# l-tamas/Fiasco

Hardware: AMD Instinct MI355X
Metric: grayscale frames/sec encoded (higher is better)
Workload: dtype f32

## Files before the change

fiasco_amd/csrc/hip/enc_layout.inc:

```

static bool long_basis(const fa_wfa *w)
{
    if (!w) return false;
    if (w->basis_states > FC_MAXBASIS) return true;
    for (unsigned s = 0; s < w->basis_states; s++)
        for (unsigned l = 0; l < 2; l++) {
            unsigned e = 0;
            while (e < 6 && FA_INTO(w, s, l, e) != FA_NO_EDGE) e++;
            if (e > FA_MAXEDGES) return true;
        }
    return false;
}
static size_t bx_bytes(const fa_wfa *w) { return 16 + (size_t) w->basis_states * 80 + 72; }

static bool needs_hm_variant(const fa_cparams *cp)
{
    return cp->rpf.mantissa_bits > 5 || cp->dc_rpf.mantissa_bits > 5 || cp->d_rpf.mantissa_bits > 5 || cp->d_dc_rpf.mantissa_bits > 5;
}

static bool needs_gm_variant(const fa_job *job)
{
    const fa_cparams *cp = &job->cp;
    const bool delta_used = cp->prediction || job->frame_type != FA_I_FRAME;
    return cp->pool_kind != FA_POOL_RLE || cp->coeff_kind != FA_COEFF_ADAPTIVE
           || (delta_used && (cp->d_pool_kind != FA_POOL_RLE || cp->d_coeff_kind != FA_COEFF_ADAPTIVE));
}

static bool needs_big_variant(const fa_cparams *cp, const fa_wfa *basis)
{
    if (needs_hm_variant(cp)) return true;
    if (cp->prediction) return true;
    if (long_basis(basis)) return true;
    if (basis)
        for (unsigned s = 0; s < basis->basis_states; s++)
            for (unsigned l = 0; l < 2; l++)
                for (unsigned e = 0; e < 6 && FA_INTO(basis, s, l, e) != FA_NO_EDGE; e++)
                    if (e >= 3) return true;
    unsigned dcs = 1u << (1 + cp->dc_rpf.mantissa_bits), sy = 1u << (1 + cp->rpf.mantissa_bits);
    return cp->lc_min_level <= cp->images_level || cp->lc_max_level > 10 || cp->max_elements > 3
           || cp->second_domain_block || cp->check_for_underflow || cp->check_for_overflow || cp->full_search
           || (cp->lc_max_level - cp->lc_min_level + 1) * sy + dcs > FC_MAXCOEFF
           || (cp->level - cp->lc_min_level + 3 + cp->lc_max_level - cp->lc_min_level)
              * ((32 + 2 * ((cp->lc_max_level - cp->lc_min_level + 1) * sy + dcs) + 15) / 16) > FC_SNAP16_WIDE;
}

static bool needs_wide_variant(const fa_cparams *cp)
{
    unsigned dcs = 1u << (1 + cp->dc_rpf.mantissa_bits), sy = 1u << (1 + cp->rpf.mantissa_bits);
    const unsigned n16 = (32 + 2 * ((cp->lc_max_level - cp->lc_min_level + 1) * sy + dcs) + 15) / 16;
    const unsigned depths = cp->level - cp->lc_min_level + 3;
    return depths - 1 > FC_MAXDEPTH_NARROW
           || (depths + cp->lc_max_level - cp->lc_min_level) * n16 > FC_SNAP16_NARROW
           || depths * 4 * ((2 * cp->limit_level + 3) / 4) > FC_SNAPTM_NARROW;
}


struct Layout {
    size_t gram, gcol, diag, ipis, d5, d4, img, imgT, imgT4, norms, num, den, est, ipdo, used, tree, into, weight,
           final_d, level_of_state, domain_type, x, y, ycol, pool_states, pos, hits, ycol0, snap, pix16, total;
    size_t ipis_alt, d5_alt, d4_alt, pix_save, sv_gram, sv_img, sv_auto;
    size_t mv, past, future, mc_fwd, mc_bwd, pix_chroma;
    size_t coop;
    size_t bx;
    size_t gq, lginv;
    int    max_save;
};

static Layout make_layout(int P, int PA, int NL, int NS, int NA, int NI, int il, int low, size_t npix,
                          int max_save, int inter, int plevels, int color, bool tri, bool hm, int gm_states = 0)
{
    Layout L;
    memset(&L, 0, sizeof L);
    size_t o = 0;
    L.max_save = max_save;
#define CARVE(field, bytes) do { L.field = o; o = align_up(o + (bytes), 256); } while (0)
    CARVE(gram, tri ? (size_t) NL * ((size_t) P * (P + 1) / 2 + P) * 4 : (size_t) NL * P * P * 4);
    CARVE(gcol, tri ? (size_t) NL * FC_TRI_HOT * P * 4 : 0);
    CARVE(diag, (size_t) NL * P * 4);
    CARVE(ipis, (size_t) NS * P * 4);
    CARVE(d5, (size_t) NA * P * 4);
    CARVE(d4, low ? (size_t) 2 * NA * P * 4 : 0);
    CARVE(img, (size_t) P * NI * 4);
    CARVE(imgT, ((size_t) 1 << il) * P * 4);
    CARVE(imgT4, low ? ((size_t) 1 << (il - 1)) * P * 4 : 0);
    CARVE(norms, (size_t) NS * 4);
    CARVE(num, (size_t) P * 4);
    CARVE(den, (size_t) P * 4);
    CARVE(est, (size_t) P * 4);
    CARVE(ipdo, (size_t) FC_MAXED * P * 4);
    CARVE(used, (size_t) P);
    CARVE(tree, (size_t) 2 * PA * 2);
    CARVE(into, (size_t) 12 * PA * 2);
    CARVE(weight, (size_t) 12 * PA * 4);
    CARVE(final_d, (size_t) PA * 4);
    CARVE(level_of_state, (size_t) PA);
    CARVE(domain_type, (size_t) PA);
    CARVE(x, (size_t) 2 * PA * 2);
    CARVE(y, (size_t) 2 * PA * 2);
    CARVE(ycol, (size_t) 2 * PA);
    CARVE(mv, inter ? (size_t) 10 * PA * 2 : 0);
    CARVE(pool_states, (size_t) (P + 8) * 2);
    CARVE(pos, (size_t) (PA + 8) * 2);
    CARVE(hits, (size_t) (PA + 8) * 4);
    CARVE(ycol0, (size_t) 2 * PA);
    const size_t n16max = FC_N16(hm ? FC_MAXCOEFF_HM : FC_MAXCOEFF_BIG_STD);
    CARVE(snap, max_save ? (size_t) (FC_MAXDEPTH_BIG * 5 * n16max + FC_MAXDEPTH_BIG * 2 * 28) * 16
                         : (size_t) 26 * 2 * n16max * 16);
    CARVE(ipis_alt, max_save ? (size_t) NS * P * 4 : 0);
    CARVE(d5_alt, max_save ? (size_t) NA * P * 4 : 0);
    CARVE(d4_alt, max_save && low ? (size_t) 2 * NA * P * 4 : 0);
    CARVE(pix_save, max_save ? (size_t) (4096 + 128) * 4 : 0);
    CARVE(sv_gram, (size_t) max_save * NL * P * 4);
    CARVE(sv_img, (size_t) max_save * (NI + 48 + NL) * 4);
    CARVE(sv_auto, (size_t) max_save * sizeof(FcSavedRow));
    CARVE(past, inter ? npix * 2 : 0);
    CARVE(future, inter == 2 ? npix * 2 : 0);
    CARVE(mc_fwd, inter ? (size_t) plevels * 1024 * 4 : 0);
    CARVE(mc_bwd, inter ? (size_t) plevels * 1024 * 4 : 0);
    CARVE(pix_chroma, inter && color ? npix / 3 * 2 * 2 : 0);
    CARVE(coop, FC_COOP_HDR + ((size_t) (NS + 1) << il) * 4);
    CARVE(bx, FC_BX_BYTES);
    CARVE(gq, gm_states ? (size_t) FC_GQ_SLOTS * P * 2 : 0);
    CARVE(lginv, gm_states ? ((size_t) gm_states + 2) * 8 : 0);
    CARVE(pix16, npix * 2);
#undef CARVE
    L.total = o;
    return L;
}

static int device_supported(const fa_job *job, char *why, size_t n)
{
    const fa_cparams *cp = &job->cp;
    const bool window_reachable = (int) cp->p_max_level >= (int) cp->lc_min_level;
    if (job->frame_type != FA_I_FRAME && window_reachable
        && (!job->past || (job->frame_type == FA_B_FRAME && !job->future) || cp->search_range != 16)) {
        snprintf(why, n, "Motion search without a reference frame (frame pattern).");
        return 0;
    }
    if ((cp->prediction || job->frame_type != FA_I_FRAME) && (int) cp->p_max_level - (int) cp->lc_min_level + 1 > 9) {
        snprintf(why, n, "prediction over more than 9 block levels is not supported by the device coder (levels %u .. %u, frame type %d)",
                 cp->lc_min_level, cp->p_max_level, job->frame_type);
        return 0;
    }
    if (cp->images_level != 5 || cp->lc_min_level < 4) {
        snprintf(why, n, "device coder needs images_level 5 and min block level >= 4");
        return 0;
    }
    if (cp->lc_max_level > 12) { snprintf(why, n, "max block level > 12 is not supported by the device coder"); return 0; }
    if (cp->max_elements > 5) { snprintf(why, n, "more than 5 vectors per block are not supported by the device coder"); return 0; }
    {
        unsigned dcs = 1u << (1 + cp->dc_rpf.mantissa_bits), sy = 1u << (1 + cp->rpf.mantissa_bits);
        if ((cp->lc_max_level - cp->lc_min_level + 1) * sy + dcs > FC_MAXCOEFF_HM) {
            snprintf(why, n, "coefficient model too large for the device coder "
                             "(block levels x mantissa symbols > %d)", FC_MAXCOEFF_HM);
            return 0;
        }
    }
    if (cp->rpf.mantissa_bits > 8 || cp->dc_rpf.mantissa_bits > 8 || cp->d_rpf.mantissa_bits > 8 || cp->d_dc_rpf.mantissa_bits > 8) {
        snprintf(why, n, "RPF mantissa > 8 bits is not supported by the device coder");
        return 0;
    }
    if (long_basis(job->wfa)) {
        const fa_wfa *w = job->wfa;
        if (bx_bytes(w) > FC_BX_BYTES) { snprintf(why, n, "initial basis too large for the device coder"); return 0; }
        for (unsigned r = 0; r < w->basis_states * 2; r++) {
            unsigned e = r * 6;
            while (e < w->basis_states * 12 && w->into[e] != FA_NO_EDGE) e++;
            if (e >= w->basis_states * 12) { snprintf(why, n, "edge lists of the initial basis run on into the coder's states"); return 0; }
        }
    }
    return 1;
}
```

fiasco_amd/csrc/hip/enc_stage.inc:

```


struct FrameSlot {
    int      job;
    char    *base = nullptr;
    size_t   bytes = 0;
    int      slab_dev = -1;
    int      P = 0, PA = 0;
    int      floorP = 0, floorPA = 0;
    Layout   L;
    DevFrame F;
    bool     staged = false, done = false, big = false, rejected = false;
    bool     hm = false;
    bool     gm = false;
    std::vector<double> lginv_host;
    bool     wide_only = false;
    bool     tri = false;
    bool     borrow = false;
    bool     spec = false;
    std::vector<uint8_t> ycol_host;
    std::vector<int32_t> bx_host;
    const int16_t *ext_pix = nullptr;
    const int16_t *ext_next = nullptr;
    const fa_image *src = nullptr;
};
// ... 10 lines not shown
    int  ncu = 256;
    std::vector<size_t>   batch;
    std::vector<DevFrame> hf;
    FcTrace *d_trace = nullptr;
    bool inflight = false, launch_failed = false, broken = false;
    int  good = 0;
    std::vector<std::pair<size_t, size_t>> to_unpack;
    char  *pinned = nullptr;
    size_t pinned_bytes = 0;
    char  *d_pack[2] = { nullptr, nullptr };
    size_t d_pack_bytes[2] = { 0, 0 }, pack_need = 0;
    int    parity = 0;
    bool   packed = false, copy_pending = false;
    std::vector<size_t> pack_off;
    hipStream_t cstream = nullptr;
    char  *up_host = nullptr;
    size_t up_host_bytes = 0;
    bool   up_host_shared = false;
    char  *up_dev[2] = { nullptr, nullptr };
    size_t up_dev_bytes[2] = { 0, 0 };
    int    up_parity = 0;
    bool   up_pending = false;
    hipStream_t ustream = nullptr;
    hipEvent_t  ev_up = nullptr;
    char  *ic_tab = nullptr, *d_ic = nullptr;
    size_t ic_cap = 0;
    hipEvent_t  ev_ic = nullptr;
    char  *peer_buf = nullptr;
    size_t peer_bytes = 0;
    char   ic_failed[200] = "";
    int       lender0 = -1;
    Layout    qL;
    int       qP = 0, qPA = 0;
    bool      qbig = false, qtri = false;
    size_t    lenders = 0, borrowers = 0, lender_cap = 0;
    char     *qpix = nullptr;
    size_t    qpix_bytes = 0, qpix_used = 0;
    unsigned long long *d_ring = nullptr;
    size_t    ring_n = 0;
    unsigned *d_queue = nullptr;
    unsigned *d_ptrmask = nullptr;
    bool      ptrmask_ready = false;
    bool      no_coop = false, no_coop_done = false;
    FcCoop    coop_hdr;
    int       specG = 0;
    int       specH[2] = { 0, 0 };
    bool      no_app = false;
    DevFrame *d_vframes = nullptr;
    size_t    vframes_n = 0;
    char     *d_spec = nullptr;
    size_t    d_spec_bytes = 0, spec_ctl_span = 0;
    std::vector<size_t> spec_frames;
    size_t    spec_first[2] = { 0, 0 }, spec_n[2] = { 0, 0 };
};

static Build build_of(const Staged *S, const FrameSlot &fs, bool few)
{
    const bool wide_only = fs.P > 12 * 256 || fs.wide_only;
    if (fs.spec && S->specG >= 2 && !fs.borrow && !fs.tri && !fs.big && fs.P <= 12 * 1024)
        return wide_only ? B_SPEC_WIDE : B_SPEC;
    if (fs.gm) return B_BIG_GM;
    if (fs.hm) return B_BIG_HM;
    if (fs.tri) return B_WIDE_TRI;
    return (Build) ((fs.big ? B_BIG : B_DEFAULT) + (few || wide_only ? 1 : 0));
}

static size_t frames_per_cu(const FrameSlot &fs)
{
    static std::atomic<int> cache[N_BUILDS];
    const Build b = fs.gm ? B_BIG_GM : fs.hm ? B_BIG_HM
                  : (Build) ((fs.big ? B_BIG : B_DEFAULT) + (fs.P > 12 * 256 || fs.wide_only ? 1 : 0));
    int occ = cache[b].load(std::memory_order_relaxed);
    if (!occ) {
        occ = k_build[b].occupancy();
        if (occ < 1) occ = 1;
        cache[b].store(occ, std::memory_order_relaxed);
    }
    return (size_t) occ;
}

static inline const fa_image *slot_image(const Staged *S, const FrameSlot &fs)
{
    return fs.src ? fs.src : S->jobs[fs.job].image;
}

static void fill_frame(FrameSlot &fs, const fa_job *job)
{
    const fa_cparams *cp = &job->cp;
    const fa_wfa *w = job->wfa;
    DevFrame &F = fs.F;
    const Layout &L = fs.L;
    char *base = fs.base;
    memset(&F, 0, sizeof F);
    F.price = cp->price;
    F.lc_min = (int) cp->lc_min_level; F.lc_max = (int) cp->lc_max_level;
    F.images_level = (int) cp->images_level; F.max_elements = (int) cp->max_elements;
    const bool bxl = long_basis(w);
    {
        unsigned live = cp->max_elements;
        for (unsigned st = 0; st < (bxl ? 0u : w->basis_states); st++)
            for (unsigned l = 0; l < 2; l++) {
                unsigned e = 0;
                while (e < 6 && FA_INTO(w, st, l, e) != FA_NO_EDGE) e++;
                if (e > live) live = e;
            }
        F.maxe_live = (int) live;
    }
    F.level = (int) cp->level; F.width = (int) job->image->width; F.height = (int) job->image->height;
    F.pool_max = (int) cp->pool_max_states; F.limit_states = (int) cp->limit_states;
    F.ML = (int) cp->limit_level;
    F.rpf_mant = (int) cp->rpf.mantissa_bits; F.dc_mant = (int) cp->dc_rpf.mantissa_bits;
    F.rpf_range = cp->rpf.range; F.dc_range = cp->dc_rpf.range;
    F.P = fs.P; F.PA = fs.PA;
    F.gram_ls = fs.tri ? (unsigned) ((size_t) fs.P * (fs.P + 1) / 2 + fs.P) : (unsigned) fs.P * (unsigned) fs.P;
    F.color = job->image->color ? 1 : 0;
    F.chroma_cl_cap = (int) knob_int("FIASCO_AMD_CLMAX", 0);
    F.chroma_sparse = !fa_knob("FIASCO_AMD_CHROMA_FULL") && (cp->pool_kind == FA_POOL_RLE || cp->pool_kind == FA_POOL_ADAPTIVE || cp->pool_kind == FA_POOL_BASIS);
    F.chroma_max = (int) cp->chroma_max_states;
    F.chroma_decrease = cp->chroma_decrease;
    F.plane = (unsigned long long) job->image->width * job->image->height;
    F.gl0 = (int) (cp->lc_min_level < cp->images_level ? cp->lc_min_level : cp->images_level);
    F.NL = (int) cp->lc_max_level - F.gl0 + 1;
    F.second_domain_block = cp->second_domain_block ? 1 : 0;
    F.check_underflow = cp->check_for_underflow ? 1 : 0;
    F.check_overflow = cp->check_for_overflow ? 1 : 0;
    F.full_search = cp->full_search ? 1 : 0;
    F.NS = (int) fa_size_of_tree(cp->products_level);
    F.NA = 1 << (cp->lc_max_level - cp->images_level);
    F.NI = (int) fa_size_of_tree(cp->images_level);
    F.dcs = 1 << (1 + F.dc_mant); F.sy = 1 << (1 + F.rpf_mant);
    F.coeff_size = (F.lc_max - F.lc_min + 1) * F.sy + F.dcs;
    F.coeff_nt = F.lc_max - F.lc_min + 2;
    F.basis_states = (int) w->basis_states;
    F.bx = bxl ? (const int *) (base + L.bx) : nullptr;
    F.gm_pool[0] = (int) cp->pool_kind; F.gm_pool[1] = (int) cp->d_pool_kind;
    F.gm_coeff[0] = (int) cp->coeff_kind; F.gm_coeff[1] = (int) cp->d_coeff_kind;
    F.gq = fs.gm ? (int16_t *) (base + L.gq) : nullptr;
    F.lginv = fs.gm ? (const double *) (base + L.lginv) : nullptr;
    for (unsigned s = 0; s < (bxl ? 0u : w->basis_states); s++) {
        F.b_final[s] = w->final_distribution[s];
        F.b_dtype[s] = w->domain_type[s];
        for (int l = 0; l < 2; l++) {
            F.b_tree[s][l] = FA_TREE(w, s, l);
            for (int e = 0; e < 6; e++) {
                F.b_into[s][l][e] = FA_INTO(w, s, l, e);
                F.b_weight[s][l][e] = FA_WEIGHT(w, s, l, e);
                if (FA_INTO(w, s, l, e) == FA_NO_EDGE) break;
            }
        }
    }
    F.pix16 = (const int16_t *) (base + L.pix16);
    F.gram = (float *) (base + L.gram); F.diag = (float *) (base + L.diag);
    F.ipis = (float *) (base + L.ipis); F.d5 = (float *) (base + L.d5);
    F.gcol = (float *) (base + L.gcol);
    F.d4 = (float *) (base + L.d4); F.imgT4 = (float *) (base + L.imgT4);
    F.img = (float *) (base + L.img); F.imgT = (float *) (base + L.imgT);
    F.norms = (float *) (base + L.norms);
    F.num = (float *) (base + L.num); F.den = (float *) (base + L.den);
    F.est = (float *) (base + L.est); F.ipdo = (float *) (base + L.ipdo);
    F.used = (uint8_t *) (base + L.used);
    F.tree = (int16_t *) (base + L.tree); F.into = (int16_t *) (base + L.into);
    F.weight = (float *) (base + L.weight); F.final_d = (float *) (base + L.final_d);
    F.level_of_state = (uint8_t *) (base + L.level_of_state);
    F.domain_type = (uint8_t *) (base + L.domain_type);
    F.x = (uint16_t *) (base + L.x); F.y = (uint16_t *) (base + L.y);
    F.ycol = (uint8_t *) (base + L.ycol);
    F.ycol0 = job->ycol_carry ? (const uint8_t *) (base + L.ycol0) : nullptr;
    F.pool_states = (int16_t *) (base + L.pool_states);
    F.pos = (int16_t *) (base + L.pos);
    F.hits = (int *) (base + L.hits);
    F.snap_hbm = fs.big ? (void *) (base + L.snap) : nullptr;
    F.l2_keys = g_l2.d_keys; F.l2_vals = g_l2.d_vals; F.l2_mask = g_l2.mask;
    const int inter = job->frame_type != FA_I_FRAME;
    F.pred_on = cp->prediction || inter ? 1 : 0;
    F.pred_root = job->image->color ? inter : (cp->prediction || inter ? 1 : 0);
    F.search_range = (int) cp->search_range;
    F.mv = (int16_t *) (base + L.mv);
    F.past = (const int16_t *) (base + L.past); F.future = (const int16_t *) (base + L.future);
    F.coop = (FcCoop *) (base + L.coop);
    F.mc_fwd = (float *) (base + L.mc_fwd); F.mc_bwd = inter ? (float *) (base + L.mc_bwd) : nullptr;
    F.pix_chroma = (int16_t *) (base + L.pix_chroma);
    F.frame_type = job->frame_type;
    F.p_min = (int) cp->p_min_level; F.p_max = (int) cp->p_max_level;
    F.d_rpf_mant = (int) cp->d_rpf.mantissa_bits; F.d_dc_mant = (int) cp->d_dc_rpf.mantissa_bits;
    F.d_rpf_range = cp->d_rpf.range; F.d_dc_range = cp->d_dc_rpf.range;
    F.d_dcs = 1 << (1 + F.d_dc_mant); F.d_sy = 1 << (1 + F.d_rpf_mant);
    F.d_coeff_size = (F.lc_max - F.lc_min + 1) * F.d_sy + F.d_dcs;
    F.ipis_alt = (float *) (base + L.ipis_alt); F.d5_alt = (float *) (base + L.d5_alt);
    F.d4_alt = (float *) (base + L.d4_alt); F.pix_save = (float *) (base + L.pix_save);
    F.sv_gram = (float *) (base + L.sv_gram); F.sv_img = (float *) (base + L.sv_img);
    F.sv_auto = (FcSavedRow *) (base + L.sv_auto);
    F.max_save = L.max_save;
    F.slab_base = base; F.slab_bytes = L.total;
}

static void slot_layout(Staged *S, FrameSlot &fs)
{
    const fa_job *job = &S->jobs[fs.job];
    const fa_cparams *cp = &job->cp;
    int il = (int) cp->images_level;
    int low = cp->lc_min_level < cp->images_level;
    int NL = (int) (cp->lc_max_level - (low ? cp->lc_min_level : cp->images_level) + 1);
    int NS = (int) fa_size_of_tree(cp->products_level);
    int NA = 1 << (cp->lc_max_level - cp->images_level);
    int NI = (int) fa_size_of_tree(cp->images_level);
    size_t npix = (size_t) job->image->width * job->image->height;
    const int bands = job->image->color ? 3 : 1;
    int max_save = 0;
    const int inter = job->frame_type;
    if (cp->prediction || inter) {
        int span = (int) cp->p_max_level - (int) cp->lc_min_level + 1;
        max_save = 1 << (span < 1 ? 1 : span > 9 ? 9 : span);
    }
    fs.L = make_layout(fs.P, fs.PA, NL, NS, NA, NI, il, low, npix * bands, max_save, inter,
                       (int) cp->p_max_level - (int) cp->p_min_level + 1, job->image->color ? 1 : 0, fs.tri, fs.hm || fs.gm,
                       fs.gm ? (int) cp->limit_states : 0);
}


static bool queue_eligible(const Staged *S, const FrameSlot &fs)
{
    const fa_job *job = &S->jobs[fs.job];
    return job->frame_type == FA_I_FRAME && !job->ycol_carry && !fs.spec && !long_basis(job->wfa) && !fs.hm && !fs.gm && !fa_knob("FIASCO_AMD_NO_QUEUE");
}

static bool queue_layout(const Staged *S, const FrameSlot &fs)
{
    if (S->lender0 < 0) return false;
    return fs.P == S->qP && fs.PA == S->qPA && fs.big == S->qbig && fs.tri == S->qtri
           && memcmp(&fs.L, &S->qL, sizeof(Layout)) == 0;
}

static int stage_borrower(Staged *S, FrameSlot &fs, size_t frames_left)
{
    fa_job *job = &S->jobs[fs.job];
    const FrameSlot &ref = S->slots[S->lender0];
    const size_t npix = (size_t) job->image->width * job->image->height;
    const int bands = job->image->color ? 3 : 1;
    const size_t need = align_up(npix * bands * 2, 256);
    if (!S->qpix && !fs.ext_pix) {
        size_t bytes = need * frames_left;
        if (hipMalloc((void **) &S->qpix, bytes) != hipSuccess) { S->qpix = nullptr; (void) hipGetLastError(); return 0; }
        S->qpix_bytes = bytes; S->qpix_used = 0;
    }
    if (!fs.ext_pix && S->qpix_used + need > S->qpix_bytes) return 0;
    fs.base = ref.base;
    fill_frame(fs, job);
    fs.base = nullptr; fs.bytes = 0;
    fs.borrow = true;
    if (fs.ext_pix) {
        fs.F.pix16 = fs.ext_pix;
        S->borrowers++;
        fs.staged = true;
        return 1;
    }
    fs.ext_pix = (const int16_t *) (S->qpix + S->qpix_used);
    fs.F.pix16 = fs.ext_pix;
    for (int b = 0; b < bands; b++)
        if (hipMemcpyAsync(S->qpix + S->qpix_used + (size_t) b * npix * 2, slot_image(S, fs)->pixels[b], npix * 2,
                           hipMemcpyHostToDevice, S->stream) != hipSuccess) {
            snprintf(job->errmsg, sizeof job->errmsg, "HIP error: pixel upload failed");
            fs.borrow = false; fs.ext_pix = nullptr;
            return 0;
        }
    S->qpix_used += need;
    S->borrowers++;
    fs.staged = true;
    return 1;
}

static bool upload_reference(Staged *S, const FrameSlot &fs, const fa_image *ref, size_t off, int here)
{
    const fa_job *job = &S->jobs[fs.job];
    const size_t npix = (size_t) job->image->width * job->image->height;
    const int bands = job->image->color ? 3 : 1;
    for (int b = 0; b < bands; b++)
        if ((ref->dev && ref->dev_id == here
             ? hipMemcpyAsync(fs.base + off + (size_t) b * npix * 2, (const int16_t *) ref->dev + (size_t) b * npix, npix * 2,
                              hipMemcpyDeviceToDevice, S->stream)
             : hipMemcpyAsync(fs.base + off + (size_t) b * npix * 2, ref->pixels[b], npix * 2,
                              hipMemcpyHostToDevice, S->stream)) != hipSuccess)
            return false;
    return true;
}

static int stage_slot(Staged *S, FrameSlot &fs)
{
    fa_job *job = &S->jobs[fs.job];
    const fa_cparams *cp = &job->cp;
    const size_t npix = (size_t) job->image->width * job->image->height;
    const int bands = job->image->color ? 3 : 1;
    slot_layout(S, fs);
    fs.base = slab_acquire(fs.L.total, &fs.bytes, &fs.slab_dev);
    if (fs.base && fa_knob("FIASCO_AMD_POISON"))
        (void) hipMemsetAsync(fs.base, (int) knob_int("FIASCO_AMD_POISON", 0), fs.L.total, S->stream);
    if (!fs.base) {
        snprintf(job->errmsg, sizeof job->errmsg, "out of HBM: frame needs %.2f GiB", fs.L.total / 1073741824.0);
        return 0;
    }
    auto give_up = [&](const char *msg) {
        snprintf(job->errmsg, sizeof job->errmsg, "%s", msg);
        slab_release(fs.base, fs.bytes, fs.slab_dev); fs.base = nullptr;
        return 0;
    };
    fill_frame(fs, job);
    const bool hmx = fs.hm || fs.gm;
// ... 324 lines not shown
```

fiasco_amd/csrc/hip/fc_config.inc:

```

#ifndef FC_VARIANT_WIDE
#define FC_VARIANT_WIDE 0
#endif
#if FC_VARIANT_WIDE
#ifndef FC_WIDE_B
#define FC_WIDE_B 512
#endif
#define B       FC_WIDE_B
#if defined(FC_VARIANT_BIG) && FC_VARIANT_BIG
#define FC_KREG 12
#elif !defined(FC_KREG)
#define FC_KREG (9216 / FC_WIDE_B)
#endif
#else
#define B       FC_BLOCK
#define FC_KREG 12
#endif
#ifndef FC_VARIANT_BIG
#define FC_VARIANT_BIG 0
#endif
#if FC_HM && !(FC_VARIANT_BIG && FC_VARIANT_WIDE)
#error "FC_HM is a variant of the 512-thread big build"
#endif
#if FC_GM && !FC_HM
#error "FC_GM is a variant of the FC_HM build"
#endif
#if FC_VARIANT_BIG
#if FC_GM
#define FC_KERNEL    fiasco_frame_kernel_big_gm
#define FC_LAUNCH    fc_launch_big_gm
#define FC_OCCUPANCY fc_occupancy_big_gm
#elif FC_HM
#define FC_KERNEL    fiasco_frame_kernel_big_hm
#define FC_LAUNCH    fc_launch_big_hm
#define FC_OCCUPANCY fc_occupancy_big_hm
#elif FC_VARIANT_WIDE
#define FC_KERNEL    fiasco_frame_kernel_big_wide
#define FC_LAUNCH    fc_launch_big_wide
#define FC_OCCUPANCY fc_occupancy_big_wide
#else
#define FC_KERNEL    fiasco_frame_kernel_big
#define FC_LAUNCH    fc_launch_big
#define FC_OCCUPANCY fc_occupancy_big
#endif
#define FC_PIXELS    4096
#define FC_NIP       4
#define FC_CLMAX     2048
#define FC_WG_PER_CU (FC_VARIANT_WIDE ? 1 : 2)
#else
#if FC_VARIANT_WIDE
#if defined(FC_SPEC) && FC_SPEC
#define FC_KERNEL    fiasco_frame_kernel_spec_wide
#define FC_LAUNCH    fc_launch_spec_wide
#define FC_OCCUPANCY fc_occupancy_spec_wide
#define FC_SPEC_SLOT_BYTES fc_spec_slot_bytes_wide
#elif defined(FC_GRAM_TRI) && FC_GRAM_TRI
#define FC_KERNEL    fiasco_frame_kernel_wide_tri
#define FC_LAUNCH    fc_launch_wide_tri
#define FC_OCCUPANCY fc_occupancy_wide_tri
#else
#define FC_KERNEL    fiasco_frame_kernel_wide
#define FC_LAUNCH    fc_launch_wide
#define FC_OCCUPANCY fc_occupancy_wide
#endif
#elif defined(FC_SPEC) && FC_SPEC
#define FC_KERNEL    fiasco_frame_kernel_spec
#define FC_LAUNCH    fc_launch_spec
#define FC_OCCUPANCY fc_occupancy_spec
#define FC_SPEC_SLOT_BYTES fc_spec_slot_bytes
#else
#define FC_KERNEL    fiasco_frame_kernel
#define FC_LAUNCH    fc_launch
#define FC_OCCUPANCY fc_occupancy
#endif
#define FC_PIXELS    1024
#define FC_NIP       2
#define FC_CLMAX     768
#ifndef FC_WG_PER_CU
#define FC_WG_PER_CU (FC_VARIANT_WIDE ? 1 : 4)
#endif
#endif
#ifndef FC_SPEC
#define FC_SPEC 0
#endif
#define SPEC_THR 1.2f
#define FC_D5T (!FC_VARIANT_BIG)
#if FC_D5T
#define D5_AT(P, NA, a, s) ((unsigned) (s) * (unsigned) (NA) + (unsigned) ((a) & 1) * ((unsigned) (NA) >> 1) + ((unsigned) (a) >> 1))
#else
#define D5_AT(P, NA, a, s) ((unsigned) (a) * (unsigned) (P) + (unsigned) (s))
#endif
#define FC_PRIO_ROTATE (!FC_VARIANT_BIG && !FC_VARIANT_WIDE && !FC_SPEC)
#define FC_PRIO_SHIFT 20
#define MAXED   FC_MAXED
#define FC_MAXE (FC_NIP + 1)
#define NOEDGE  (-1)
#define RANGE_  (-1)
#define MAXCOSTS 1e20f
#define BIGF    3.0e38f
#define MIN_NORM 2e-3f

enum { OP_DONE = 0, OP_INIT_RANGE, OP_APPROX, OP_IPIS_INCR, OP_APPEND, OP_NOP, OP_CHROMA,
       OP_PRED_SETUP, OP_PRED_FINISH, OP_NORMS, OP_MC_SEARCH, OP_SPEC_CKPT };
enum { PH_ENTER = 0, PH_AFTER_INIT, PH_AFTER_LC, PH_CHILD, PH_CHILD2, PH_CHILD_RET, PH_DECIDE,
       PH_AFTER_APPEND, PH_PRED_BEGIN, PH_PRED_RECURSE, PH_PRED_RET, PH_PRED_DONE, PH_PRED_MC2, PH_PRED_GO,
       PH_SPEC_END };
enum { MV_NONE = 0, MV_FORWARD = 1, MV_BACKWARD = 2, MV_INTERPOLATED = 3 };
#ifdef FC_DUP_OP
#define FC_DUP(o, call) do { if ((o) == FC_DUP_OP) { __syncthreads(); call; } } while (0)
#else
#define FC_DUP(o, call) do { } while (0)
#endif
#if FC_VARIANT_BIG
#define FC_DEPTH FC_MAXDEPTH_BIG
#elif FC_VARIANT_WIDE
#define FC_DEPTH FC_MAXDEPTH
#else
#define FC_DEPTH FC_MAXDEPTH_NARROW
#endif
```

fiasco_amd/csrc/hip/fc_tables.inc:

```


#if FC_VARIANT_BIG
#define ACT_IPIS(F, sh) ((sh).par.ipis)
#define ACT_D5(F, sh)   ((sh).par.d5)
#define ACT_D4(F, sh)   ((sh).par.d4)
#elif FC_SPEC
#define ACT_IPIS(F, sh) ((sh).par.ipis)
#define ACT_D5(F, sh)   ((sh).par.d5)
#define ACT_D4(F, sh)   ((F).d4)
#else
#define ACT_IPIS(F, sh) ((F).ipis)
#define ACT_D5(F, sh)   ((F).d5)
#define ACT_D4(F, sh)   ((F).d4)
#endif

__device__ __forceinline__ int table_states(const Sh &sh) { return sh.band ? sh.ystates : sh.states; }

struct AutoTabs {
    GLOBAL_AS const int16_t *tree, *into;
    GLOBAL_AS const float   *weight;
    GLOBAL_AS const uint8_t *domain_type;
    int PA;
};

__device__ __forceinline__ void auto_tabs(const DevFrame &F, AutoTabs &t)
{
    t.tree = uniform_ptr((const int16_t *) F.tree); t.into = uniform_ptr((const int16_t *) F.into);
    t.weight = uniform_ptr((const float *) F.weight);
    t.domain_type = uniform_ptr((const uint8_t *) F.domain_type);
    t.PA = __builtin_amdgcn_readfirstlane(F.PA);
}

template <int E> struct EdgeRowsT {
    int   tree[2], rd[2][E];
    float rw[2][E];
    int   dt;
};
typedef EdgeRowsT<FC_MAXE> EdgeRows;

template <int E> __device__ __forceinline__ void load_edge_rows(const AutoTabs &T, int s, EdgeRowsT<E> &r)
{
    unsigned us = (unsigned) s;
    asm volatile("" : "+v"(us));
    r.dt = ldg(T.domain_type, us);
#pragma unroll
    for (int l = 0; l < 2; l++) {
        r.tree[l] = ldg(T.tree, us + (unsigned) (l * T.PA));
#pragma unroll
        for (int e = 0; e < E; e++) {
            r.rd[l][e] = ldg(T.into, us + (unsigned) ((l * 6 + e) * T.PA));
            r.rw[l][e] = ldg(T.weight, us + (unsigned) ((l * 6 + e) * T.PA));
        }
    }
}

template <int E> __device__ __noinline__ void op_ipis_t(const DevFrame &__restrict__ F, Sh &__restrict__ sh, int image, int address, int level, int from, int lv_first)
{
    const int tid = threadIdx.x, il = F.images_level;
    const int P = __builtin_amdgcn_readfirstlane(F.P), states = __builtin_amdgcn_readfirstlane(table_states(sh));
    image = __builtin_amdgcn_readfirstlane(image); address = __builtin_amdgcn_readfirstlane(address);
    level = __builtin_amdgcn_readfirstlane(level); from = __builtin_amdgcn_readfirstlane(from);
    GLOBAL_AS float *const ipis = uniform_ptr(ACT_IPIS(F, sh));
    GLOBAL_AS const float *const d5 = uniform_ptr((const float *) ACT_D5(F, sh));
    AutoTabs T;
    auto_tabs(F, T);
    lv_first = __builtin_amdgcn_readfirstlane(lv_first);
    for (int lv = lv_first > il + 1 ? lv_first : il + 1; lv <= level; lv++) {
        int delta = level - lv;
        int cnt = 1 << delta;
        int slot0 = ((image + 1) << delta) - 1;
        int adr0 = address << delta;
#if FC_D5T
        const bool first = lv == il + 1;
        const unsigned NAu = (unsigned) __builtin_amdgcn_readfirstlane(F.NA), NAh = NAu >> 1;
        const bool vec4 = first && cnt >= 4 && (NAh & 3u) == 0;
        GLOBAL_AS const float *src0 = first ? d5 : ipis + (size_t) (slot0 * 2 + 1) * P;
#else
        GLOBAL_AS const float *src0 = (lv == il + 1) ? d5 + (size_t) (adr0 * 2) * P
                                                     : ipis + (size_t) (slot0 * 2 + 1) * P;
#endif
        int s = from + tid;
#if FC_VARIANT_BIG
        if (F.bx) {
            const BxView V = bx_view(F);
            for (int i = tid; i < V.nb * cnt; i += B) {
                const int bs = i / cnt, j = i - bs * cnt;
                if (bs < from || !V.dtype[bs]) continue;
                float acc = 0;
                for (int l = 0; l < 2; l++) {
                    int dom;
                    for (int e = (bs * 2 + l) * 6; (dom = V.into[e]) != NOEDGE; e++)
                        acc += V.w[e] * ldg(src0, (unsigned) dom + (unsigned) ((j * 2 + l) * P));
                }
                stg(ipis, (unsigned) bs + (unsigned) ((slot0 + j) * P), acc);
            }
            if (from < V.nb) s = V.nb + tid;
        }
#endif
        EdgeRowsT<E> nx;
        if (s < states) load_edge_rows(T, s, nx);
        for (; s < states; s += B) {
            const EdgeRowsT<E> cur = nx;
            if (s + B < states) load_edge_rows(T, s + B, nx);
            const bool tabled = cur.dt && !DEAD(sh, s);
            if (!tabled) continue;
            int   idx[2][E + 1];
            float wt[2][E + 1];
            unsigned msk[2];
#pragma unroll
            for (int l = 0; l < 2; l++) {
                int k = cur.tree[l];
                msk[l] = k != RANGE_ ? 1u : 0u;
                idx[l][0] = k != RANGE_ ? k : 0;
                wt[l][0] = 1.0f;
                bool live = true;
#pragma unroll
                for (int e = 0; e < E; e++) {
                    live = live && cur.rd[l][e] != NOEDGE;
                    idx[l][e + 1] = live ? cur.rd[l][e] : 0;
                    wt[l][e + 1] = live ? cur.rw[l][e] : 0.0f;
                    msk[l] |= live ? (2u << e) : 0u;
                }
            }
            constexpr int JG = 4;
            for (int j0 = 0; j0 < cnt; j0 += JG) {
                float v[JG][2][E + 1];
#if FC_D5T
                if (vec4) {
                    typedef float f4 __attribute__((ext_vector_type(4)));
#pragma unroll
                    for (int l = 0; l < 2; l++)
#pragma unroll
                        for (int i = 0; i <= E; i++) {
                            const unsigned o = (unsigned) idx[l][i] * NAu + (unsigned) l * NAh + (unsigned) (adr0 + j0);
                            const f4 q = *(GLOBAL_AS const f4 *) (src0 + o);
                            v[0][l][i] = q.x; v[1][l][i] = q.y; v[2][l][i] = q.z; v[3][l][i] = q.w;
                        }
                } else if (first) {
#pragma unroll
                    for (int jj = 0; jj < JG; jj++)
#pragma unroll
                        for (int l = 0; l < 2; l++)
#pragma unroll
                            for (int i = 0; i <= E; i++) {
                                const int jc = j0 + jj < cnt ? j0 + jj : cnt - 1;
                                v[jj][l][i] = ldg(src0, (unsigned) idx[l][i] * NAu + (unsigned) l * NAh + (unsigned) (adr0 + jc));
                            }
                } else
#endif
#pragma unroll
                for (int jj = 0; jj < JG; jj++)
#pragma unroll
                    for (int l = 0; l < 2; l++)
#pragma unroll
                        for (int i = 0; i <= E; i++) {
                            const int jc = j0 + jj < cnt ? j0 + jj : cnt - 1;
                            v[jj][l][i] = ldg(src0, (unsigned) idx[l][i] + (unsigned) ((jc * 2 + l) * P));
                        }
#pragma unroll
                for (int jj = 0; jj < JG; jj++) {
                    if (j0 + jj >= cnt) break;
                    float acc = 0;
#pragma unroll
                    for (int l = 0; l < 2; l++) {
                        if (msk[l] & 1u) acc += v[jj][l][0];
#pragma unroll
                        for (int i = 1; i <= E; i++)
                            if ((msk[l] >> i) & 1u) acc += wt[l][i] * v[jj][l][i];
                    }
                    stg(ipis, (unsigned) s + (unsigned) ((slot0 + j0 + jj) * P), acc);
                }
            }
        }
        __syncthreads();
    }
}

__device__ __forceinline__ void op_ipis(const DevFrame &__restrict__ F, Sh &__restrict__ sh, int image, int address, int level, int from,
                                        int lv_first = 0)
{
#if FC_VARIANT_BIG
    if (F.maxe_live <= 3) { op_ipis_t<3>(F, sh, image, address, level, from, lv_first); return; }
#endif
    op_ipis_t<FC_MAXE>(F, sh, image, address, level, from, lv_first);
}

__device__ void op_d5(const DevFrame &__restrict__ F, Sh &__restrict__ sh, int from, int to, int na, int n4, int abase = 0, int pxoff = 0)
{
    const int tid = threadIdx.x, P = __builtin_amdgcn_readfirstlane(F.P);
    GLOBAL_AS float *const D5 = uniform_ptr(ACT_D5(F, sh));
    GLOBAL_AS const float *const imgT = uniform_ptr((const float *) F.imgT);
    GLOBAL_AS const uint8_t *const dtype = uniform_ptr((const uint8_t *) F.domain_type);
    for (int s = from + tid; s < to; s += B) {
        if (DEAD(sh, s) || !ldg(dtype, (unsigned) s)) continue;
        float v[32];
#pragma unroll
        for (int k = 0; k < 32; k++) v[k] = ldg(imgT, (unsigned) (k * P + s));
        typedef float f2 __attribute__((ext_vector_type(2)));
#if FC_D5T
        const unsigned NAu = (unsigned) __builtin_amdgcn_readfirstlane(F.NA), NAh = NAu >> 1;
        int a = 0;
        if ((NAh & 3u) == 0)
            for (; a + 8 <= na; a += 8) {
                f2 ip[4] = { { 0.0f, 0.0f }, { 0.0f, 0.0f }, { 0.0f, 0.0f }, { 0.0f, 0.0f } };
#pragma unroll
                for (int k = 0; k < 32; k++) {
                    f2 vv = { v[k], v[k] };
#pragma unroll
                    for (int u = 0; u < 4; u++) {
                        f2 px = { sh.pixels[(a + 2 * u) * 32 + k], sh.pixels[(a + 2 * u) * 32 + 32 + k] };
                        ip[u] = ip[u] + px * vv;
                    }
                }
                typedef float f4 __attribute__((ext_vector_type(4)));
                const f4 ev = { ip[0].x, ip[1].x, ip[2].x, ip[3].x }, od = { ip[0].y, ip[1].y, ip[2].y, ip[3].y };
                const unsigned o = (unsigned) s * NAu + ((unsigned) a >> 1);
                *(GLOBAL_AS f4 *) (D5 + o) = ev;
                *(GLOBAL_AS f4 *) (D5 + o + NAh) = od;
            }
        for (; a < na; a += 2) {
            f2 ip = { 0.0f, 0.0f };
#pragma unroll
            for (int k = 0; k < 32; k++) {
                f2 px = { sh.pixels[a * 32 + k], sh.pixels[a * 32 + 32 + k] };
                f2 vv = { v[k], v[k] };
                ip = ip + px * vv;
            }
            stg(D5, D5_AT(P, NAu, a, s), ip.x);
            if (a + 1 < na) stg(D5, D5_AT(P, NAu, a + 1, s), ip.y);
        }
#else
        for (int a = 0; a < na; a += 2) {
            f2 ip = { 0.0f, 0.0f };
#pragma unroll
            for (int k = 0; k < 32; k++) {
                f2 px = { sh.pixels[pxoff + a * 32 + k], sh.pixels[pxoff + a * 32 + 32 + k] };
                f2 vv = { v[k], v[k] };
                ip = ip + px * vv;
            }
            stg(D5, (unsigned) ((abase + a) * P + s), ip.x);
            if (a + 1 < na) stg(D5, (unsigned) ((abase + a + 1) * P + s), ip.y);
        }
#endif
#if FC_VARIANT_BIG
        if (F.gl0 < F.images_level) {
            float *const D4 = ACT_D4(F, sh);
#pragma unroll
            for (int k = 0; k < 16; k++) v[k] = F.imgT4[(size_t) k * P + s];
            for (int a = 0; a < n4; a++) {
                float ip = 0;
#pragma unroll
                for (int k = 0; k < 16; k++) ip += sh.pixels[pxoff + a * 16 + k] * v[k];
                D4[(size_t) (2 * abase + a) * P + s] = ip;
            }
        }
#endif
    }
}

#if FC_VARIANT_BIG
__device__ __forceinline__ float *coop_pixels(FcCoop *c) { return (float *) ((char *) c + FC_COOP_HDR); }

__device__ void coop_share(const DevFrame &__restrict__ F, Sh &__restrict__ sh, int level, int from, unsigned member, unsigned W, int D)
{
    const int il = F.images_level, sub = level - D, nasub = 1 << (sub - il);
    for (int j = (int) member; j < (1 << D); j += (int) W)
        op_d5(F, sh, from, table_states(sh), nasub, 2 * nasub, j * nasub, j << sub);
    __syncthreads();
    for (int j = (int) member; j < (1 << D); j += (int) W)
        op_ipis(F, sh, (1 << D) - 1 + j, j, sub, from);
}

__device__ int coop_publish(DevFrame &__restrict__ F, Sh &__restrict__ sh, int level, int from)
{
    const int tid = threadIdx.x, il = F.images_level;
    const unsigned W = sh.coopW;
    FcCoop *c = F.coop;
    if (W < 2 || !c) return 0;
    const int D = sh.coopD;
    if (level - il < D + sh.coop_minsub) return 0;
    float *gp = coop_pixels(c);
    for (int i = tid; i < (1 << level); i += B) gp[i] = sh.pixels[i];
    asm volatile("s_waitcnt vmcnt(0)" ::: "memory");
    __syncthreads();
    if (tid == 0) {
        c->level = level; c->from = from; c->to = table_states(sh);
        c->ipis = sh.par.ipis; c->d5 = sh.par.d5; c->d4 = sh.par.d4;
        __builtin_amdgcn_fence(__ATOMIC_RELEASE, "agent");
        asm volatile("s_waitcnt vmcnt(0)" ::: "memory");
        sh.coop_seq++;
        __hip_atomic_store(&c->seq, sh.coop_seq, __ATOMIC_RELAXED, __HIP_MEMORY_SCOPE_AGENT);
    }
    return D;
}

__device__ void coop_finish(DevFrame &__restrict__ F, Sh &__restrict__ sh, int level, int from, int D)
{
    const int tid = threadIdx.x;
    const unsigned W = sh.coopW;
    FcCoop *c = F.coop;
    coop_share(F, sh, level, from, 0, W, D);
    __syncthreads();
    if (tid == 0) {
        const unsigned want = sh.coop_seq * (W - 1);
        const unsigned long long t_give_up = wall_clock64() + sh.coop_ticks;
        while (__hip_atomic_load(&c->done, __ATOMIC_RELAXED, __HIP_MEMORY_SCOPE_AGENT) < want) {
            if (wall_clock64() > t_give_up) { sh.failed = FC_ERR_COOP; break; }
            __builtin_amdgcn_s_sleep(4);
        }
        __builtin_amdgcn_fence(__ATOMIC_ACQUIRE, "agent");
    }
    __syncthreads();
}

__device__ void coop_helper(DevFrame &__restrict__ F, Sh &__restrict__ sh, unsigned member, unsigned W)
{
    const int tid = threadIdx.x;
    FcCoop *c = F.coop;
    unsigned seen = 0;
    if (!c) return;
    for (;;) {
        if (tid == 0) {
            const unsigned long long t_give_up = wall_clock64() + FC_COOP_WAIT_TICKS;
            int go = 0;
// ... 263 lines not shown
```

fiasco_amd/csrc/hip/frame_coder.h:

```cpp
#ifndef FRAME_CODER_H
#define FRAME_CODER_H
#include <stdint.h>

#define FC_MAXED    5
#define FC_BLOCK    256
#define FC_MAXDEPTH 22
#define FC_MAXDEPTH_BIG 32
#define FC_MAXDEPTH_NARROW 18
#define FC_SNAP16_NARROW 480
#define FC_SNAP16_WIDE   840
#define FC_SNAPTM_NARROW 988
#define FC_SNAPTM_WIDE   1092
#define FC_MAXSAVE  512
#define FC_MAXCOEFF 224
#ifndef FC_HM
#define FC_HM 0
#endif
#ifndef FC_GM
#define FC_GM 0
#endif
enum { FC_PK_ADAPTIVE = 0, FC_PK_CONSTANT = 1, FC_PK_BASIS = 2, FC_PK_UNIFORM = 3, FC_PK_RLE = 4, FC_PK_RLE_NO_CHROMA = 5 };
enum { FC_CK_ADAPTIVE = 0, FC_CK_UNIFORM = 1 };
#define FC_GQ_SLOTS (2 + FC_MAXDEPTH_BIG * 5)
#define FC_MAXCOEFF_BIG_STD 640
#define FC_MAXSYM_STD   64
#define FC_MAXCOEFF_HM  5120
#define FC_MAXSYM_HM    512
#define FC_MAXCOEFF_BIG (FC_HM ? FC_MAXCOEFF_HM : FC_MAXCOEFF_BIG_STD)
#define FC_MAXSYM       (FC_HM ? FC_MAXSYM_HM : FC_MAXSYM_STD)
#define FC_N16(coeffs)  ((32 + 2 * (coeffs) + 15) / 16)
#define FC_N16MAX       FC_N16(FC_MAXCOEFF_BIG)
#define FC_MAXBASIS 16
#define FC_BX_BYTES (64 * 1024)
#ifndef FC_TRI_HOT
#define FC_TRI_HOT  8
#endif

enum { FC_OK = 1, FC_ERR_STATES = 2, FC_ERR_CAPACITY = 3, FC_ERR_NOROOT = 4, FC_ERR_INTERNAL = 5,
       FC_ERR_QUEUE = 6,
       FC_ERR_COOP = 7 };
struct FcCoop {
    unsigned seq;
    unsigned done;
    unsigned quit;
    unsigned depth;
    int      level, from, to;
    int      minsub;
    float   *ipis, *d5, *d4;
    unsigned long long done_ticks;
};
#define FC_COOP_HDR 128
#define FC_COOP_WAIT_TICKS 3000000000ull
#define FC_COOP_DONE_TICKS 500000000ull
#define FC_QUEUE_WAIT_TICKS 60000000000ull

struct FcTrace;
typedef struct DevFrame {
    float    price;
    int      lc_min, lc_max, images_level, max_elements;
    int      maxe_live;
    int      gl0;
    int      second_domain_block;
    int      check_underflow, check_overflow, full_search;
    int      level, width, height;
    int      pool_max, limit_states, ML;
    int      rpf_mant, dc_mant;
    float    rpf_range, dc_range;
    int      P;
    unsigned gram_ls;
    int      PA;
    int      color;
    int      chroma_sparse;
    int      chroma_cl_cap;
    int      chroma_max;
    float    chroma_decrease;
    unsigned long long plane;
    int      NL, NS, NA, NI;
    int      coeff_size, coeff_nt, dcs, sy;
    int      basis_states;
    int16_t  b_tree[FC_MAXBASIS][2];
    int16_t  b_into[FC_MAXBASIS][2][6];
    float    b_weight[FC_MAXBASIS][2][6];
    float    b_final[FC_MAXBASIS];
    uint8_t  b_dtype[FC_MAXBASIS];
    const int *bx;
    int      gm_pool[2], gm_coeff[2];
    int16_t *gq;
    const double *lginv;
    const int16_t *pix16;
    float   *gram, *diag, *ipis, *d5, *img, *imgT, *norms;
    float   *gcol;
    float   *d4, *imgT4;
    float   *num, *den, *est, *ipdo;
    uint8_t *used;
    int16_t *tree, *into;
    float   *weight, *final_d;
    uint8_t *level_of_state, *domain_type;
    uint16_t *x, *y;
    uint8_t *ycol;
    const uint8_t *ycol0;
    void    *snap_hbm;
    int      pred_root;
    int      pred_on;
    int      frame_type;
    int      p_min, p_max;
    int      d_rpf_mant, d_dc_mant;
    float    d_rpf_range, d_dc_range;
    int      d_coeff_size, d_dcs, d_sy;
    float   *ipis_alt, *d5_alt, *d4_alt;
    float   *pix_save;
    float   *sv_gram;
    float   *sv_img;
    struct FcSavedRow *sv_auto;
    int      max_save;
    const int16_t *past, *future;
    float   *mc_fwd, *mc_bwd;
    int16_t *mv;
    int16_t *pix_chroma;
    int      search_range;
    int16_t *pool_states;
    int16_t *pos;
    int     *hits;
    const void *pack_src;
    void    *pack_dst;
    unsigned pack_bytes;
    const unsigned *l2_keys;
    const double   *l2_vals;
    unsigned        l2_mask;
    int      status;
    int      states, root_state;
    FcCoop  *coop;
    int      ystates_out;
    float    costs, err, tree_bits, matrix_bits, weights_bits;
    float    c_costs[2], c_err[2], c_tree_bits[2], c_matrix_bits[2], c_weights_bits[2];
    int      lc_min_out;
    unsigned long long bytes_mp, bytes_img, bytes_gram;
    unsigned long long n_mp, n_steps, n_blocks, n_appends, n_fulleval;
    unsigned long long t_init, t_approx, t_ipis, t_append, t_serial, t_total;
    unsigned long long t_mpA, t_mpB, n_blockevals;
    unsigned long long dbg[8];
    struct FcTrace *trace;
    int      trace_cap, trace_n;
    char    *slab_base;
    unsigned long long slab_bytes;
    struct FcSpecCtl *spec;
    int      spec_role, spec_G;
    int      spec_tb;
    int      spec_cap;
    int      spec_T;
} DevFrame;

#define FC_DESC_WORDS ((sizeof(DevFrame) + 7) / 8)

#define FC_SPEC_W      16
#define FC_SPEC_TEMPS  16
#define FC_SPEC_MAXG   8
#define FC_SPEC_R      24
typedef struct FcSpecCtl {
    unsigned next;
    unsigned epoch;
    unsigned done;
    unsigned committed;
    unsigned adopting;
    unsigned busy;
    unsigned slot_bytes;
    unsigned slot_seq[FC_SPEC_W];
    unsigned verdict[FC_SPEC_W];
    unsigned long long n_tasks, n_confirmed, n_wrong, n_timeout, n_inline, t_wait;
    unsigned long long n_tab_used, n_tab_missed;
    unsigned long long n_adopted;
    unsigned s_pub;
    unsigned tab_free;
    unsigned blk_cur;
    unsigned chroma_ready, tab_next, ystates;
    unsigned n_tabs;
    unsigned n_blocks;
    unsigned tab_stride;
    unsigned tab_wait;
    unsigned long long off_blocks, off_tabs;
    unsigned tab_seq[FC_SPEC_R];
    unsigned tab_s[FC_SPEC_R];
    unsigned tab_epoch[FC_SPEC_R];
    unsigned app_H;
    unsigned app_min;
    unsigned app_wait;
    unsigned app_seq;
    unsigned app_done;
    unsigned app_off;
    unsigned app_dbg;
    int      app_s, app_flim;
    int      app_n[2], app_c[2], app_idx[2][FC_MAXED + 1];
    float    app_w[2][FC_MAXED + 1];
    unsigned long long n_app_dealt, t_app_wait;
} FcSpecCtl;

typedef struct FcSavedRow {
    int16_t  tree[2], into[2][6];
    float    weight[2][6];
    float    final_d;
    uint16_t x[2], y[2];
    int16_t  pos;
    int16_t  mv[2][5];
    uint8_t  level, dtype, ycol[2], tables;
} FcSavedRow;

typedef struct FcTrace {
    int   seq, level, image, D, states, nedges;
    float cost, err, mbits, wbits;
    short into[6];
    float w[5];
} FcTrace;

#endif
```

Measured before the change: 610.1.

## Add state-major transposed inner-product buffer for vectorized child-level ipis reads

Adds a new ipt buffer that stores each level's inner products in state-major, even/odd-split order as they are computed. The next level reads this buffer with contiguous float4/float2 loads instead of strided scalar loads from ipis. It is enabled by default for non-big, non-spec variants. The cost is an extra NA*P float buffer and additional global stores on every level below lc_max.

```diff
diff --git a/fiasco_amd/csrc/hip/enc_layout.inc b/fiasco_amd/csrc/hip/enc_layout.inc
--- a/fiasco_amd/csrc/hip/enc_layout.inc
+++ b/fiasco_amd/csrc/hip/enc_layout.inc
@@ -56,7 +56,7 @@
 
 
 struct Layout {
-    size_t gram, gcol, diag, ipis, d5, d4, img, imgT, imgT4, norms, num, den, est, ipdo, used, tree, into, weight,
+    size_t gram, gcol, diag, ipis, d5, ipt, d4, img, imgT, imgT4, norms, num, den, est, ipdo, used, tree, into, weight,
            final_d, level_of_state, domain_type, x, y, ycol, pool_states, pos, hits, ycol0, snap, pix16, total;
     size_t ipis_alt, d5_alt, d4_alt, pix_save, sv_gram, sv_img, sv_auto;
     size_t mv, past, future, mc_fwd, mc_bwd, pix_chroma;
@@ -79,6 +79,7 @@
     CARVE(diag, (size_t) NL * P * 4);
     CARVE(ipis, (size_t) NS * P * 4);
     CARVE(d5, (size_t) NA * P * 4);
+    CARVE(ipt, (size_t) NA * P * 4);
     CARVE(d4, low ? (size_t) 2 * NA * P * 4 : 0);
     CARVE(img, (size_t) P * NI * 4);
     CARVE(imgT, ((size_t) 1 << il) * P * 4);
diff --git a/fiasco_amd/csrc/hip/enc_stage.inc b/fiasco_amd/csrc/hip/enc_stage.inc
--- a/fiasco_amd/csrc/hip/enc_stage.inc
+++ b/fiasco_amd/csrc/hip/enc_stage.inc
@@ -186,6 +186,7 @@
     F.pix16 = (const int16_t *) (base + L.pix16);
     F.gram = (float *) (base + L.gram); F.diag = (float *) (base + L.diag);
     F.ipis = (float *) (base + L.ipis); F.d5 = (float *) (base + L.d5);
+    F.ipt = (float *) (base + L.ipt);
     F.gcol = (float *) (base + L.gcol);
     F.d4 = (float *) (base + L.d4); F.imgT4 = (float *) (base + L.imgT4);
     F.img = (float *) (base + L.img); F.imgT = (float *) (base + L.imgT);
diff --git a/fiasco_amd/csrc/hip/fc_config.inc b/fiasco_amd/csrc/hip/fc_config.inc
--- a/fiasco_amd/csrc/hip/fc_config.inc
+++ b/fiasco_amd/csrc/hip/fc_config.inc
@@ -85,6 +85,12 @@
 #endif
 #define SPEC_THR 1.2f
 #define FC_D5T (!FC_VARIANT_BIG)
+#ifndef FC_IPT
+#define FC_IPT (!FC_VARIANT_BIG && !FC_SPEC)
+#endif
+#if FC_IPT && !FC_D5T
+#error "FC_IPT goes with the state-major level-images_level dots (FC_D5T)"
+#endif
 #if FC_D5T
 #define D5_AT(P, NA, a, s) ((unsigned) (s) * (unsigned) (NA) + (unsigned) ((a) & 1) * ((unsigned) (NA) >> 1) + ((unsigned) (a) >> 1))
 #else
diff --git a/fiasco_amd/csrc/hip/fc_tables.inc b/fiasco_amd/csrc/hip/fc_tables.inc
--- a/fiasco_amd/csrc/hip/fc_tables.inc
+++ b/fiasco_amd/csrc/hip/fc_tables.inc
@@ -1,3 +1,4 @@
+#include "ipt_layout.h"
 
 
 #if FC_VARIANT_BIG
@@ -56,12 +57,20 @@
 
 template <int E> __device__ __noinline__ void op_ipis_t(const DevFrame &__restrict__ F, Sh &__restrict__ sh, int image, int address, int level, int from, int lv_first)
 {
+#if FC_IPT
+    const int tid = threadIdx.x, il = __builtin_amdgcn_readfirstlane(F.images_level);
+#else
     const int tid = threadIdx.x, il = F.images_level;
+#endif
     const int P = __builtin_amdgcn_readfirstlane(F.P), states = __builtin_amdgcn_readfirstlane(table_states(sh));
     image = __builtin_amdgcn_readfirstlane(image); address = __builtin_amdgcn_readfirstlane(address);
     level = __builtin_amdgcn_readfirstlane(level); from = __builtin_amdgcn_readfirstlane(from);
     GLOBAL_AS float *const ipis = uniform_ptr(ACT_IPIS(F, sh));
     GLOBAL_AS const float *const d5 = uniform_ptr((const float *) ACT_D5(F, sh));
+#if FC_IPT
+    GLOBAL_AS float *const ipt = uniform_ptr(F.ipt);
+    const int lc_max = __builtin_amdgcn_readfirstlane(F.lc_max);
+#endif
     AutoTabs T;
     auto_tabs(F, T);
     lv_first = __builtin_amdgcn_readfirstlane(lv_first);
@@ -73,8 +82,16 @@
 #if FC_D5T
         const bool first = lv == il + 1;
         const unsigned NAu = (unsigned) __builtin_amdgcn_readfirstlane(F.NA), NAh = NAu >> 1;
+#if FC_IPT
+        const unsigned n_lv = ipt_n(lc_max, lv);
+        GLOBAL_AS const float *src0 = first ? d5 : (GLOBAL_AS const float *) ipt;
+        const unsigned Pu = (unsigned) P, rs = first ? NAu : 2u * n_lv;
+        const unsigned lb[2] = { first ? 0u : ipt_row(Pu, NAu, 2u * n_lv, 0u) + ipt_src_col(n_lv, 0u, 0u),
+                                 first ? NAh : ipt_row(Pu, NAu, 2u * n_lv, 0u) + ipt_src_col(n_lv, 1u, 0u) };
+#else
         const bool vec4 = first && cnt >= 4 && (NAh & 3u) == 0;
         GLOBAL_AS const float *src0 = first ? d5 : ipis + (size_t) (slot0 * 2 + 1) * P;
+#endif
 #else
         GLOBAL_AS const float *src0 = (lv == il + 1) ? d5 + (size_t) (adr0 * 2) * P
                                                      : ipis + (size_t) (slot0 * 2 + 1) * P;
@@ -125,6 +142,39 @@
             constexpr int JG = 4;
             for (int j0 = 0; j0 < cnt; j0 += JG) {
                 float v[JG][2][E + 1];
+#if FC_IPT
+                unsigned ob[2][E + 1];
+#pragma unroll
+                for (int l = 0; l < 2; l++)
+#pragma unroll
+                    for (int i = 0; i <= E; i++) ob[l][i] = ((unsigned) idx[l][i] * rs + lb[l] + (unsigned) (adr0 + j0)) * 4u;
+                if (cnt >= 4) {
+                    typedef float f4 __attribute__((ext_vector_type(4)));
+#pragma unroll
+                    for (int l = 0; l < 2; l++)
+#pragma unroll
+                        for (int i = 0; i <= E; i++) {
+                            const f4 q = *(GLOBAL_AS const f4 *) ((GLOBAL_AS const char *) src0 + ob[l][i]);
+                            v[0][l][i] = q.x; v[1][l][i] = q.y; v[2][l][i] = q.z; v[3][l][i] = q.w;
+                        }
+                } else if (cnt == 2) {
+                    typedef float f2 __attribute__((ext_vector_type(2)));
+#pragma unroll
+                    for (int l = 0; l < 2; l++)
+#pragma unroll
+                        for (int i = 0; i <= E; i++) {
+                            const f2 q = *(GLOBAL_AS const f2 *) ((GLOBAL_AS const char *) src0 + ob[l][i]);
+                            v[0][l][i] = q.x; v[1][l][i] = q.y;
+                        }
+                } else {
+#pragma unroll
+                    for (int l = 0; l < 2; l++)
+#pragma unroll
+                        for (int i = 0; i <= E; i++)
+                            v[0][l][i] = *(GLOBAL_AS const float *) ((GLOBAL_AS const char *) src0 + ob[l][i]);
+                }
+                float res[JG];
+#else
 #if FC_D5T
                 if (vec4) {
                     typedef float f4 __attribute__((ext_vector_type(4)));
@@ -157,6 +207,7 @@
                             const int jc = j0 + jj < cnt ? j0 + jj : cnt - 1;
                             v[jj][l][i] = ldg(src0, (unsigned) idx[l][i] + (unsigned) ((jc * 2 + l) * P));
                         }
+#endif
 #pragma unroll
                 for (int jj = 0; jj < JG; jj++) {
                     if (j0 + jj >= cnt) break;
@@ -169,7 +220,24 @@
                             if ((msk[l] >> i) & 1u) acc += wt[l][i] * v[jj][l][i];
                     }
                     stg(ipis, (unsigned) s + (unsigned) ((slot0 + j0 + jj) * P), acc);
+#if FC_IPT
+                    res[jj] = acc;
+#endif
                 }
+#if FC_IPT
+                if (lv < lc_max) {
+                    const unsigned a0 = (unsigned) (adr0 + j0), row = ipt_row(Pu, NAu, n_lv, (unsigned) s);
+                    if (cnt >= 4) {
+                        typedef float f2 __attribute__((ext_vector_type(2)));
+                        const f2 ev = { res[0], res[2] }, od = { res[1], res[3] };
+                        *(GLOBAL_AS f2 *) ((GLOBAL_AS char *) ipt + (row + ipt_col(n_lv, a0)) * 4u) = ev;
+                        *(GLOBAL_AS f2 *) ((GLOBAL_AS char *) ipt + (row + ipt_col(n_lv, a0 + 1u)) * 4u) = od;
+                    } else {
+                        stg(ipt, row + ipt_col(n_lv, a0), res[0]);
+                        if (cnt == 2) stg(ipt, row + ipt_col(n_lv, a0 + 1u), res[1]);
+                    }
+                }
+#endif
             }
         }
         __syncthreads();
diff --git a/fiasco_amd/csrc/hip/frame_coder.h b/fiasco_amd/csrc/hip/frame_coder.h
--- a/fiasco_amd/csrc/hip/frame_coder.h
+++ b/fiasco_amd/csrc/hip/frame_coder.h
@@ -91,6 +91,7 @@
     float   *gram, *diag, *ipis, *d5, *img, *imgT, *norms;
     float   *gcol;
     float   *d4, *imgT4;
+    float   *ipt;
     float   *num, *den, *est, *ipdo;
     uint8_t *used;
     int16_t *tree, *into;
diff --git a/fiasco_amd/csrc/hip/ipt_layout.h b/fiasco_amd/csrc/hip/ipt_layout.h
--- /dev/null
+++ b/fiasco_amd/csrc/hip/ipt_layout.h
@@ -0,0 +1,16 @@
+#ifndef FIASCO_IPT_LAYOUT_H
+#define FIASCO_IPT_LAYOUT_H
+
+#if defined(__HIPCC__) || defined(__CUDACC__)
+#define IPT_FN __host__ __device__ inline
+#else
+#define IPT_FN inline
+#endif
+
+IPT_FN unsigned ipt_n(int lc_max, int lv) { return 1u << (lc_max - lv); }
+IPT_FN unsigned ipt_row(unsigned P, unsigned NA, unsigned n, unsigned s) { return (NA - 2u * n) * P + s * n; }
+IPT_FN unsigned ipt_col(unsigned n, unsigned a) { return (a & 1u) * (n >> 1) + (a >> 1); }
+IPT_FN unsigned ipt_src_col(unsigned n, unsigned l, unsigned a) { return l * n + a; }
+IPT_FN unsigned ipt_width(unsigned cnt) { return cnt >= 4u ? 4u : cnt; }
+
+#endif
```

Measured after the change: 617.4, median of 6. 1.2% higher.
